# cgmb/euler

Hardware: AMD Instinct MI355X
Metric: cells*steps/sec of sim_step() (frames incl. the PCG pressure projection) + pressure-solve HBM GB/s vs roofline (higher is better)
Workload: dtype f64

## Files before the change

### euler_amd/csrc/driver.hip

```cpp
#include "euler_dev.h"
#include "k_mg.h"

#include <math.h>
#include <stdarg.h>
#include <stdlib.h>
#include <string.h>

#include <vector>

int eu_launch_build_system(euler_sim* S, float dt);
int eu_launch_velocity_update(euler_sim* S, float dt, int finish);
int eu_pressure_current(euler_sim* S);
int eu_unskew(euler_sim* S, const void* skew, void* rowmajor, int elem_bytes);
int eu_unskew_fluid(euler_sim* S, const double* skew, double* rowmajor);
double* eu_current_search_direction(euler_sim* S);
int eu_launch_tile_table(euler_sim* S);
int eu_skew(euler_sim* S, const void* rowmajor, void* skew, int elem_bytes);

static thread_local char g_err[512] = "";

void eu_set_error(const char* fmt, ...) {
  va_list ap;
  va_start(ap, fmt);
  vsnprintf(g_err, sizeof(g_err), fmt, ap);
// ... 105 lines not shown
  return EULER_OK;
}

bool eu_resident_eligible(const euler_sim* S) {
  if (S->res_disabled || S->cfg.resident == EULER_RESIDENT_OFF) return false;
  if (S->cfg.precond != EULER_PRECOND_IC0_TILE || S->tile_w != 16 || S->cfg.sweep_mode == EULER_SWEEP_SIMPLE || S->cfg.dot_mode != EULER_DOT_TREE) return false;
  if (S->has_comm || S->slab_on || S->p2p_on) return false;
  const int cap = eu_resident_capacity(const_cast<euler_sim*>(S), S->cfg.pcg_precision == EULER_PCG_F32);
  if (S->cfg.pcg_precision == EULER_PCG_F32) return cap > 0 && S->geom.nbands * (S->geom.T / 16) <= 4 * cap;
  return cap > 0;
}
extern "C" int euler_resident_info(euler_sim* S, uint64_t out[3]) {
  if (!S || !out) return EULER_EINVAL;
  out[0] = eu_resident_eligible(S) ? 1 : 0; out[1] = S->res_solves; out[2] = S->res_fallbacks;
  return EULER_OK;
}

extern "C" int euler_set_option(euler_sim* S, int32_t key, int64_t value) {
  if (!S || key <= 0 || key >= EULER_OPT__COUNT) { eu_set_error("euler_set_option: unknown key %d", (int)key); return EULER_EINVAL; }
  bool ok = true;
  const char* when = nullptr;
  switch (key) {
    case EULER_OPT_P_STEPS: ok = value == 2 || value == 4 || value == 8; break;
    case EULER_OPT_SA_RUN: ok = value == 8 || value == 16 || value == 32;
      if (ok && value != 8 && (S->has_comm || eu_is_two_level(S))) when = "on a handle without a communicator, in the parity or the plain tile-local mode (the others run runs of 8)";
      break;
    case EULER_OPT_RCCL_SMALL: ok = value >= 0 && value <= 2; if (S->rccl) when = "before euler_set_comm_rccl"; break;
    case EULER_OPT_RCCL_NO_EXCHANGE: ok = value == 0 || value == 1; if (S->rccl) when = "before euler_set_comm_rccl"; break;
    case EULER_OPT_SLAB_FUSION: ok = value == 0 || value == 1; if (S->p2p_on) when = "before euler_p2p_connect"; break;
    case EULER_OPT_RESIDENT_CAP: case EULER_OPT_GRID4_MIN_CELLS: case EULER_OPT_RESIDENT_FORCE_TIMEOUT: ok = value >= 0; break;
    case EULER_OPT_MG_SPLIT_LEVEL: ok = value >= -1 && value < 12; break;
    case EULER_OPT_PROFILE_STRIDE: ok = value >= 1 && value <= 1024; break;
    case EULER_OPT_MG_SPLIT_ACTIVE: ok = false; break;
    case EULER_OPT_ADVECT_RK2: ok = value == 0 || value == 1;
      if (ok && value == 1 && S->slab_on) when = "on a whole-grid handle (row slabs: the midpoint samples reach one row beyond the ghost rows)";
      break;
    case EULER_OPT_ADVECT_MACCORMACK: ok = value == 0 || value == 1;
      if (ok && value == 1 && S->slab_on) when = "on a whole-grid handle (row slabs: the correction reads the forward result one row beyond the own rows)";
      break;
    default: ok = value == 0 || value == 1; break;
  }
  if (!ok) { eu_set_error("euler_set_option: key %d does not take the value %lld", (int)key, (long long)value); return EULER_EINVAL; }
  if (when) { eu_set_error("euler_set_option: key %d must be set %s", (int)key, when); return EULER_ESTATE; }
  HIPCHK(hipStreamSynchronize(S->stream));
  if (key == EULER_OPT_ADVECT_MACCORMACK && value == 1 && !S->mc_u) {
    float *a = nullptr, *b = nullptr;
    const size_t bytes = S->C * sizeof(float);
    if (hipMalloc((void**)&a, bytes) != hipSuccess || hipMalloc((void**)&b, bytes) != hipSuccess || hipMemset(a, 0, bytes) != hipSuccess ||
        hipMemset(b, 0, bytes) != hipSuccess) {
      if (a) (void)hipFree(a);
      if (b) (void)hipFree(b);
      (void)hipGetLastError();
      eu_set_error("euler_set_option: EULER_OPT_ADVECT_MACCORMACK needs %zu bytes of scratch", 2 * bytes);
      return EULER_ENOMEM;
    }
    S->mc_u = a; S->mc_v = b;
    S->hbm_bytes += 2 * bytes;
  }
  if (key == EULER_OPT_P_STEPS || key == EULER_OPT_SA_RUN) {
    int rcp = eu_pressure_current(S);
    if (rcp) return rcp;
  }
  S->opt[key] = value;
  if (key == EULER_OPT_P_STEPS || key == EULER_OPT_SA_RUN) S->s_ring_n = 0;
  if (key == EULER_OPT_MG_SPLIT_LEVEL) { eu_mg_split_release(S); S->opt[EULER_OPT_MG_SPLIT_ACTIVE] = 0; }
  return EULER_OK;
// ... 925 lines not shown
```

### euler_amd/csrc/k_pcg.h

```cpp
#pragma once

#include "euler_dev.h"
#include "k_mg.h"

#define COMM_CALL(expr) do { if ((expr) != 0) { eu_set_error("communicator callback failed: %s", #expr); return EULER_ECOMM; } } while (0)
#define LOC(ptr) ((ptr) + S->e_lo)
enum { SW_FACTOR = 0, SW_FORWARD = 1, SW_BACKWARD = 2 };

int eu_launch_build_system(euler_sim* S, float dt);
int eu_launch_velocity_update(euler_sim* S, float dt, int finish);
int eu_launch_band_ranges(euler_sim* S);
int eu_launch_sweep(euler_sim* S, int op, int cls, int force, int fin_qq = -1);
int eu_launch_factor_tile(euler_sim* S, int force);
int eu_launch_precond_tile(euler_sim* S, int rupd, int sweeps, int fin_dot, int force, double alpha, bool r_only = false, int zform = -1);
int eu_launch_search_apply(euler_sim* S, int it);
int eu_launch_finish_p(euler_sim* S);
int eu_launch_dot(euler_sim* S, const double* a, const double* b, int fin_op, int force);
int eu_comm_exchange(euler_sim* S, double* send_lo, double* send_hi, double* recv_lo, double* recv_hi, int count, double* small, int nsmall);
int eu_comm_finish(euler_sim* S, int fin_op, int is_max, int force);
int eu_comm_halo_two(euler_sim* S, double* a, double* b);
bool tile_recompute(const euler_sim* S);
int p_steps(const euler_sim* S);

enum { FIN_SIGMA_INIT = 0, FIN_ALPHA, FIN_RNORM, FIN_BETA, FIN_STORE_ONLY, FIN_TO_COMM };
#define FIN_VIA_P2P 0x100

static inline bool tile_fused(const euler_sim* S) { return eu_is_tile(S) && S->cfg.sweep_mode != EULER_SWEEP_SIMPLE; }
static inline bool ghost_mode(const euler_sim* S) { return S->has_comm && !S->p2p_on && tile_fused(S); }
enum { XR_ZSEND_LO = 0, XR_ZSEND_HI, XR_ZRECV_LO, XR_ZRECV_HI, XR_GS_LO0, XR_GS_LO1, XR_GS_HI0, XR_GS_HI1 };
static inline double* xrow(const euler_sim* S, int k) { return S->xrows + (size_t)k * S->xrow_len; }
static inline int sa_run(const euler_sim* S) {
  if (S->opt[EULER_OPT_SA_RUN] != 8 && !S->has_comm && !eu_is_two_level(S)) return (int)S->opt[EULER_OPT_SA_RUN];
  return 8;
}
static inline bool tile_z_recompute(const euler_sim* S) {
  return tile_recompute(S) && tile_fused(S) && !eu_is_two_level(S) && S->tile_w == 16 && !S->has_comm && !S->slab_on && S->band_lo == 0 &&
         S->opt[EULER_OPT_TILE_STORE_Z] == 0 && S->chunk_list && S->tile_table;
}
static inline int fin_or_comm(const euler_sim* S, int fin_op) {
  return S->has_comm ? (S->p2p_on ? (fin_op | FIN_VIA_P2P) : (int)FIN_TO_COMM) : fin_op;
}

#ifdef __HIPCC__
#define RED_THREADS 1024
typedef double sw_d2 __attribute__((ext_vector_type(2)));

__device__ __forceinline__ bool pcg_idle(const PcgScalars* sc) { return sc->done || !sc->nonzero; }

#define DPP_WAVE_SHL1 0x130
#define DPP_WAVE_SHR1 0x138

template <int CTRL>
__device__ __forceinline__ double wave_shift_inject(double v, double edge) {
  const int lo = __builtin_amdgcn_update_dpp(__double2loint(edge), __double2loint(v), CTRL, 0xf, 0xf, false);
  const int hi = __builtin_amdgcn_update_dpp(__double2hiint(edge), __double2hiint(v), CTRL, 0xf, 0xf, false);
  return __hiloint2double(hi, lo);
}


__device__ __forceinline__ void pcg_scalar_step(PcgScalars* sc, int op, double v) {
  switch (op) {
    case FIN_SIGMA_INIT: sc->sigma = v; break;
    case FIN_ALPHA: sc->zs = v; sc->alpha_prev = sc->alpha; sc->alpha = sc->sigma / v; sc->alpha_hist[sc->iters & 7] = sc->alpha; sc->iters += 1; break;
    case FIN_RNORM: sc->rnorm = v; if (v <= sc->tol) sc->done = 1; break;
    case FIN_BETA: sc->sigma_new = v; sc->beta = v / sc->sigma; sc->sigma = v; break;
    case FIN_TO_COMM: sc->comm_val = v; if (sc->comm_slot) *sc->comm_slot = v; break;
    default: sc->sigma_new = v; break;
  }
}

template <int NT = RED_THREADS>
// ... 129 lines not shown
  unsigned int* qq_counter;
  PcgScalars* sc_w;
};

struct TileArgs {
  SkewGeom g;
  const uint8_t* mask;
  double* pre;
  double* r;
  const double* as;
  double* z;
  int band_lo, nb_local;
  int rupd;
  int sweeps;
  int fin_dot;
  int via;
  double* part_max; double* part_dot;
  unsigned int* counter;
  const unsigned int* list;
  const double* table;
  PcgScalars* sc;
  int force;
  double alpha_arg;
  double* pair_slot;
  double *zsend_lo, *zsend_hi;
  int edge_lo, edge_hi;
  int reverse;
  double* cpart;
  int cshift;
  int cmode, cnx, cny;
  const double *gs_lo, *gs_hi;
  int zform;
  double *zhalo, *zrows;
};

__device__ __forceinline__ double factor_step(double aa, double own, double nbv) {
  const double cl = -1.0 * own, cb = -1.0 * nbv;
  double e = aa - cl * cl - cb * cb;
  if (e < 0.25 * aa) e = (aa != 0.0) ? aa : 1.0;
  return 1.0 / sqrt(e);
}

template <int CTRL>
__device__ __forceinline__ double dpp_move(double v) {
  const int lo = __builtin_amdgcn_update_dpp(0, __double2loint(v), CTRL, 0xf, 0xf, true);
  const int hi = __builtin_amdgcn_update_dpp(0, __double2hiint(v), CTRL, 0xf, 0xf, true);
  return __hiloint2double(hi, lo);
}
__device__ __forceinline__ double group_sum(double v) {
  v = v + dpp_move<0xB1>(v);
  v = v + dpp_move<0x4E>(v);
  if (MG_LG == 8) v = v + dpp_move<0x141>(v);
  return v;
}
#endif
```

### euler_amd/csrc/k_pcg.hip

```cpp
#include "k_pcg.h"

#include <cmath>
#include <vector>

template <bool IS_MAX>
__global__ __launch_bounds__(RED_THREADS) void k_reduce_final(const double* __restrict__ partial, int n, PcgScalars* sc,
                                                              int op, int force) {
  if (!force && pcg_idle(sc)) return;
  double v = 0.0;
  for (int i = threadIdx.x; i < n; i += RED_THREADS) {
    const double w = partial[i];
    if (IS_MAX) v = w > v ? w : v; else v += w;
  }
  v = IS_MAX ? block_max(v) : block_sum(v);
  if (threadIdx.x == 0) pcg_scalar_step(sc, op, v);
}

template <bool EDGES>
__global__ __launch_bounds__(RED_THREADS) void k_dot_partial(const double* __restrict__ a, const double* __restrict__ b,
                                                             const uint8_t* __restrict__ mask, size_t S,
                                                             double* __restrict__ partial, PcgScalars* sc, int force,
                                                             unsigned int* counter, int fin_op, int TS, int nb_local, int edges) {
  if (!force && pcg_idle(sc)) return;
  const size_t chunk = (((S + gridDim.x - 1) / gridDim.x) + 1) & ~(size_t)1;
// ... 491 lines not shown
      S->prof_iter = -2;
      if (int rc = eu_launch_resident(S, cap_chunks)) return rc;
      HIPCHK(hipMemcpyAsync(S->sc_host, S->sc, sizeof(PcgScalars), hipMemcpyDeviceToHost, S->stream));
      HIPCHK(hipStreamSynchronize(S->stream));
      S->res_last_chunks = S->sc_host->n_chunks; S->res_have_last = 1;
      const int err = *S->res_err;
      if (err == 0) {
        if (S->sc_host->nonzero) { S->res_solves += 1; S->pcg_fields_resident = 1; }
        return eu_launch_velocity_update(S, dt, 0);
      }
      *S->res_err = 0;
      if (S->cfg.pcg_precision == EULER_PCG_F32 && err == 2) { eu_set_error("EULER_PCG_F32: the solve's active chunks do not fit the resident solver"); return EULER_EHIP; }
      if (err != 2) { S->res_fallbacks += 1; S->res_disabled = 1; }
      S->solve_seq -= 1;
      S->lean_ok = 0;
      S->res_skip_once = 1;
      *S->sc_host = v.prev;
      return eu_launch_project(S, dt);
    }
  }
  return EULER_OK;
}

static int project_first_direction(euler_sim* S, Solve& v) {
  int rc;
  const bool tile = tile_fused(S), two_level = tile && eu_is_two_level(S);
  if (two_level && S->has_comm && !(eu_is_mg(S) && ghost_mode(S) && S->slab_on)) {
    eu_set_error("coarse-correction preconditioners with several ranks: EULER_PRECOND_IC0_TILE_MG on row slabs without mailboxes only");
    return EULER_EINVAL;
  }
  if (two_level && (rc = eu_launch_coarse_setup(S))) return rc;
  if (two_level && (rc = eu_launch_coarse_consistent(S))) return rc;
  v.zr = tile && tile_z_begin(S);
  if (tile) {
    if ((rc = eu_launch_factor_tile(S, 0))) return rc;
    if ((rc = eu_launch_precond_tile(S, 0, 1, FIN_SIGMA_INIT, 0, 0.0))) return rc;
  } else {
  if (S->cfg.precond != EULER_PRECOND_JACOBI && (rc = eu_launch_sweep(S, SW_FACTOR, KC_PRECON_FACTOR, 0))) return rc;
  if ((rc = launch_precondition(S, 0, FIN_SIGMA_INIT))) return rc;
  }
  if ((rc = ring_begin(S))) return rc;
  if (first_direction_folded(S)) {
    const PcgScalars& ps = v.prev;
    if (ps.nonzero && !(std::isfinite(ps.alpha) && std::isfinite(ps.beta) && std::isfinite(ps.rnorm) && std::isfinite(ps.sigma) && std::isfinite(ps.zs)))
      for (int k = 0; k < S->s_ring_n; ++k) HIPCHK(hipMemsetAsync(S->s_ring[k] + S->skew_off, 0, S->Sw * sizeof(double), S->stream));
  }
  else if (two_level) { if ((rc = eu_launch_coarse_search_init(S))) return rc; }
  else
  LAUNCH(S, KC_UPDATE_SEARCH, k_update_search<true>, dim3(eu_blocks(S->e_cnt, 256 * 4, 4096)), dim3(256), LOC(S->s), LOC(S->z),
         LOC(S->cellmask), S->e_cnt, S->sc, 0, 0.0);
  if (S->has_comm && eu_p2p_has_neighbour_arrays(S)) {
    const int y0 = S->band_lo > 0 ? 64 * S->band_lo : -1, y1 = S->band_hi < S->geom.nbands ? 64 * S->band_hi - 1 : -1;
    LAUNCH(S, KC_UPDATE_SEARCH, k_publish_edge_rows, dim3((S->X + 255) / 256, 2), dim3(256), S->s, S->geom, y0, y1, S->sc);
  }
  if (S->s_ring_n == 2) HIPCHK(hipMemsetAsync(LOC(S->s2), 0, S->e_cnt * sizeof(double), S->stream));
  S->s_stale = 1;
  return EULER_OK;
}

static int project_iterate(euler_sim* S, Solve& v) {
  int rc;
  HIPCHK(hipMemcpyAsync(S->sc_host, S->sc, sizeof(PcgScalars), hipMemcpyDeviceToHost, S->stream));
  HIPCHK(hipStreamSynchronize(S->stream));
  const int poll = S->cfg.pcg_poll_interval > 0 ? S->cfg.pcg_poll_interval : 8;
  const int max_it = S->cfg.max_iterations;
  const bool tile = tile_fused(S), fold0 = first_direction_folded(S);
  int it = 0, chunk = 0;
  bool stop = !S->sc_host->nonzero;
  S->s_none = stop ? 1 : 0;
  while (it < max_it && !stop) {
    int chunk_end = it + poll;
    if (!v.drain_poll && v.pred_iters > 0 && it < v.pred_iters + poll && chunk_end > v.pred_iters - 2) {
      const int lo = v.pred_iters - 2 < chunk_end ? v.pred_iters - 2 : chunk_end;
      chunk_end = lo > it + 2 ? lo : it + 2;
    }
    if (chunk_end > max_it) chunk_end = max_it;
    for (; it < chunk_end; ++it) {
      S->prof_iter = it;
      const bool fused = it > 0 || fold0;
      if (it == 0 && fold0) { S->s = S->s_ring[S->s_ring_n - 1]; S->s2 = S->s_ring[0]; }
      if ((rc = fused ? eu_launch_search_apply(S, it) : launch_apply_a_and_alpha(S, 0))) return rc;
      if (tile) {
        S->prof_iter = it;
        const int nx = it + 1, steps = S->s_ring_n;
        const bool next_odd = !(nx >= steps && nx % steps == 0);
        const int zform = v.zr && it + 1 < max_it ? (it + 2 < max_it && next_odd ? 1 : 0) : -1;
        if ((rc = eu_launch_precond_tile(S, 1, it + 1 < max_it, FIN_BETA, 0, 0.0, false, zform))) return rc;
        S->z_halo_last = zform == 1;
        v.zr_ran = v.zr_ran || zform == 1;
        continue;
      }
      S->tile_as_override = fused ? S->q : S->z;
      rc = eu_launch_precond_tile(S, 1, 0, -1, 0, 0.0, true);
      S->tile_as_override = nullptr;
      if (rc) return rc;
      if (it + 1 < max_it) {
        S->prof_iter = it + 1;
        if ((rc = launch_precondition(S, 0, FIN_BETA))) return rc;
      }
    }
    if (it < max_it && v.drain_poll) {
      HIPCHK(hipMemcpyAsync(S->sc_host, S->sc, sizeof(PcgScalars), hipMemcpyDeviceToHost, S->stream));
      HIPCHK(hipStreamSynchronize(S->stream));
      stop = S->sc_host->done != 0;
    } else
    if (it < max_it) {
      const int slot = chunk & 1;
      if (chunk > 0) {
        HIPCHK(hipEventSynchronize(S->poll_event[slot ^ 1]));
        stop = S->poll_host[slot ^ 1].done != 0;
      }
      HIPCHK(hipMemcpyAsync(&S->poll_host[slot], S->sc, sizeof(PcgScalars), hipMemcpyDeviceToHost, S->stream));
      HIPCHK(hipEventRecord(S->poll_event[slot], S->stream));
      ++chunk;
    }
  }
  return EULER_OK;
}

// ... 85 lines not shown
```

### euler_amd/csrc/k_search.hip

```cpp
#include "k_pcg.h"

#include <type_traits>

#define SA_THREADS 256
struct SaPair { sw_d2 z, so; double ez0, es0, ez1, es1; };

__device__ __forceinline__ double pick3(int t, int tb1, int tb2, double v0, double v1, double v2) {
  double v = v0;
  v = t >= tb1 ? v1 : v;
  v = t >= tb2 ? v2 : v;
  return v;
}
template <int SLAB, int PMODE, int SA_RUN, int COARSE = 0, bool STORE = true, bool ZR = false>
__global__ __launch_bounds__(SA_THREADS, (COARSE == 2 && PMODE == 1 && SLAB == 0) ? 4 : 1) void k_search_apply(const double* __restrict__ s_old, const double* __restrict__ z,
                                                             double* __restrict__ s_new, double* __restrict__ out,
                                                             const uint8_t* __restrict__ mask, SkewGeom g,
                                                             double* __restrict__ partial, PcgScalars* sc, int force,
                                                             unsigned int* counter, int fin_op, SlabNeighbours nbr,
                                                             double* __restrict__ p, double* s_new_base, double* s_old_base,
                                                             const unsigned int* __restrict__ chunk_list,
                                                             CoarseRef cref, SaHist hist, ZrArgs zr) {
  static_assert(PMODE == 1 || PMODE == 2 || PMODE == 4 || PMODE == 8, "PMODE: p is left alone (1) or takes the N fmadds that are due (the ring's length)");
  static_assert(!ZR || (SLAB == 0 && SA_RUN == 8 && COARSE == 0), "ZR: one GPU, runs of one tile, no coarse part");
  __shared__ double s_cy[COARSE == 2 ? SA_THREADS / 64 : 1][COARSE == 2 ? MG_NI + 1 : 1][64];
  __shared__ double s_ce[COARSE == 2 ? SA_THREADS / 64 : 1][COARSE == 2 ? MG_NI + 1 : 1][64];
  if (!force && pcg_idle(sc)) return;
  __shared__ sw_d2 s_ztab[ZR ? 8 : 1][64];
  if (ZR) {
    for (int k = threadIdx.x; k < 8 * 64; k += SA_THREADS) (&s_ztab[0][0])[k] = reinterpret_cast<const sw_d2*>(zr.table)[k];
    __syncthreads();
  }
  const double beta = sc->beta;
  (void)s_new_base; (void)s_old_base;
  constexpr int NPA = PMODE >= 2 ? PMODE : 2;
  double al[NPA] = {};
  if (PMODE >= 2) {
    const int k = sc->iters;
#pragma unroll
    for (int j = 0; j < NPA; ++j) al[j] = sc->alpha_hist[(k - NPA + j) & 7];
  }
  const int lane = threadIdx.x & 63;
  const int TS = g.TS, npairs = TS / 2;
  const int nb_local = (int)(g.S / ((size_t)TS * 64));
  const int cpb = (npairs + SA_RUN - 1) / SA_RUN, total = nb_local * cpb;
  const int n_waves = gridDim.x * (SA_THREADS / 64);
  const bool edge_lane = lane == 0 || lane == 63;
  double t = 0.0;
  const bool listed = chunk_list != nullptr;
  const int ntb16 = g.T / 16;
  const int todo = listed ? (int)sc->n_chunks : total;
  typedef std::integral_constant<bool, true> yes_t;
  typedef std::integral_constant<bool, false> no_t;
  for (int i = blockIdx.x * (SA_THREADS / 64) + (threadIdx.x >> 6); i < todo; i += n_waves) {
    int c = i, per = cpb;
    bool interior = false;
    if (listed) { const unsigned int ent = chunk_list[i]; interior = (ent & EU_CHUNK_INTERIOR) != 0; c = (int)(ent & ~EU_CHUNK_INTERIOR); per = ntb16; }
    const int lb = c / per, P0 = (c % per) * SA_RUN, P1 = ZR ? P0 + SA_RUN : (P0 + SA_RUN < npairs ? P0 + SA_RUN : npairs);
    const size_t bbase = (size_t)lb * TS * 64 + 2 * lane;
    auto run = [&](auto full_tag) {
      constexpr bool FULL = decltype(full_tag)::value;
      unsigned int mm[SA_RUN];
      unsigned int any = 0;
#pragma unroll
      for (int j = 0; j < SA_RUN; ++j) {
        if (FULL) mm[j] = CM_INTERIOR | (CM_INTERIOR << 8);
        else mm[j] = P0 + j < P1 ? (unsigned int)*reinterpret_cast<const unsigned short*>(mask + bbase + (size_t)(P0 + j) * 128) : 0u;
        any |= mm[j];
      }
      if (!FULL && !listed && !__ballot(((any | (any >> 8)) & CM_FLUID) != 0)) return;
      sw_d2 zz[ZR ? SA_RUN : 1];
      if (ZR) {
        sw_d2 rr[SA_RUN], pp[SA_RUN];
#pragma unroll
        for (int j = 0; j < SA_RUN; ++j) {
          rr[j] = *reinterpret_cast<const sw_d2*>(zr.r + bbase + (size_t)(P0 + j) * 128);
          pp[j] = FULL ? s_ztab[j][lane] : *reinterpret_cast<const sw_d2*>(zr.pre + bbase + (size_t)(P0 + j) * 128);
        }
        double none = 0.0;
        tile_solve<2 * SA_RUN, false>(mm, rr, pp, zz, none);
      }
      const int ztile = P0 / SA_RUN;
      const bool up_remote = SLAB == 1 && nbr.z_up && lb + 1 == nb_local, dn_remote = SLAB == 1 && nbr.z_dn && lb == 0;
      const double* ez = lane == 0 ? (dn_remote ? nbr.z_dn : z) : (up_remote ? nbr.z_up : z);
      const double* es = lane == 0 ? (dn_remote ? nbr.s_dn : s_old) : (up_remote ? nbr.s_up : s_old);
      const bool remote = lane == 0 ? dn_remote : up_remote;
      const long long e0_base = lane == 0 ? ((long long)(lb - 1) * TS + 62) * 64 + 127 : ((long long)(lb + 1) * TS - 64) * 64 + 1;
      const long long e1_base = lane == 0 ? ((long long)(lb - 1) * TS + 64) * 64 + 126 : ((long long)(lb + 1) * TS - 62) * 64;
      const unsigned int vbit = lane == 0 ? CM_DOWN : CM_UP;
      const bool ghost = SLAB == 2 && (lane == 0 ? (nbr.zrow_dn != nullptr && lb == 0) : (nbr.zrow_up != nullptr && lb + 1 == nb_local));
      const double* gz = lane == 0 ? nbr.zrow_dn : nbr.zrow_up;
      const double* gs = lane == 0 ? nbr.srow_dn : nbr.srow_up;
      double* gsn = lane == 0 ? nbr.snew_dn : nbr.snew_up;
      const int gcol = lane == 0 ? 0 : -63;
      const double* zrow = ZR ? zr.rows + (long long)(lane == 0 ? 2 * lb - 1 : 2 * lb + 2) * zr.X : nullptr;
      double cy0 = 0.0, cy1 = 0.0, cy2 = 0.0, ce0 = 0.0, ce1 = 0.0, ce2 = 0.0;
      double (*cyv)[64] = s_cy[COARSE == 2 ? threadIdx.x >> 6 : 0];
      double (*cev)[64] = s_ce[COARSE == 2 ? threadIdx.x >> 6 : 0];
      int ctb1 = 0x7fffffff, ctb2 = 0x7fffffff, cJb = 0;
      (void)cJb;
      if (COARSE == 2) {
        cJb = (2 * (P0 - 1) - lane - MG_G0 / 2) >> MG_LOG;
        ctb1 = MG_G0 * (cJb + 1) + lane + MG_G0 / 2;
        const int row = (cref.band0 + lb) * 64 + lane;
        const int hi_ = cref.nx - 1;
        int i0, i1;
        double fy;
        mg_cell_w(row, cref.ny, i0, i1, fy);
        const double* y0 = cref.y + (size_t)i0 * cref.nx;
        const double* y1 = cref.y + (size_t)i1 * cref.nx;
#pragma unroll
        for (int q = 0; q <= MG_NI; ++q) { const int c = cJb + q < 0 ? 0 : (cJb + q < hi_ ? cJb + q : hi_); cyv[q][lane] = mg_rows(y0[c], y1[c], fy); }
#pragma unroll
        for (int q = 0; q <= MG_NI; ++q) cev[q][lane] = 0.0;
        if (edge_lane) {
          const int re = row + (lane == 0 ? -1 : 1);
          if (re >= 0 && re < MG_G0 * cref.ny) {
            mg_cell_w(re, cref.ny, i0, i1, fy);
            y0 = cref.y + (size_t)i0 * cref.nx; y1 = cref.y + (size_t)i1 * cref.nx;
#pragma unroll
            for (int q = 0; q <= MG_NI; ++q) { const int c = cJb + q < 0 ? 0 : (cJb + q < hi_ ? cJb + q : hi_); cev[q][lane] = mg_rows(y0[c], y1[c], fy); }
          }
        }
      }
      auto p0y = [&](int t, double (*av)[64]) __attribute__((always_inline)) {
        const double f = (double)((t - lane - MG_G0 / 2) & (MG_G0 - 1)) * (1.0 / MG_G0);
        int m = t >= ctb1 ? ((t - ctb1) >> MG_LOG) + 1 : 0;
        m = m < MG_NI - 1 ? m : MG_NI - 1;
        return mg_lerp_x(av[m][lane], av[m + 1][lane], f);
      };
      if (COARSE == 1) {
        const int xa = 2 * (P0 - 1) - lane, Ja = (xa > 0 ? xa : 0) >> cref.shift;
        const int row = (cref.band0 + lb) * 64 + lane;
        const size_t I = (size_t)(row >> cref.shift) * cref.nx;
        ctb1 = ((Ja + 1) << cref.shift) + lane;
        ctb2 = ((Ja + 2) << cref.shift) + lane;
        cy0 = Ja < cref.nx ? cref.y[I + Ja] : 0.0;
        cy1 = Ja + 1 < cref.nx ? cref.y[I + Ja + 1] : 0.0;
        cy2 = Ja + 2 < cref.nx ? cref.y[I + Ja + 2] : 0.0;
        if (edge_lane) {
          const int re = row + (lane == 0 ? -1 : 1);
          const bool inside = re >= 0 && (re >> cref.shift) < cref.ny;
          const size_t Ie = (size_t)((inside ? re : row) >> cref.shift) * cref.nx;
          ce0 = (inside && Ja < cref.nx) ? cref.y[Ie + Ja] : 0.0;
          ce1 = (inside && Ja + 1 < cref.nx) ? cref.y[Ie + Ja + 1] : 0.0;
          ce2 = (inside && Ja + 2 < cref.nx) ? cref.y[Ie + Ja + 2] : 0.0;
        }
      }
      auto load_pair = [&](int P, SaPair& d, unsigned int m) __attribute__((always_inline)) {
        d.ez0 = d.es0 = d.ez1 = d.es1 = 0.0;
        if (P < 0 || P >= npairs) { d.z = sw_d2{0.0, 0.0}; d.so = sw_d2{0.0, 0.0}; return; }
        if (ZR) {
          const int j = P - P0;
          if (j >= 0 && j < SA_RUN) d.z = zz[j >= 0 && j < SA_RUN ? j : 0];
          else if (j < 0) d.z = sw_d2{0.0, zr.halo[((size_t)lb * ntb16 + ztile - 1) * 128 + 64 + lane]};
          else d.z = sw_d2{ztile + 1 < ntb16 ? zr.halo[((size_t)lb * ntb16 + ztile + 1) * 128 + lane] : 0.0, 0.0};
        } else {
          d.z = *reinterpret_cast<const sw_d2*>(z + bbase + (size_t)P * 128);
        }
        d.so = *reinterpret_cast<const sw_d2*>(s_old + bbase + (size_t)P * 128);
        if (edge_lane) {
          if ((m & CM_FLUID) && (m & vbit)) {
            const long long k = e0_base + (long long)P * 128;
            if (ZR) { d.ez0 = zrow[2 * P + gcol]; d.es0 = s_old[k]; }
            else if (SLAB == 2 && ghost) { d.ez0 = gz[2 * P + gcol]; d.es0 = gs[2 * P + gcol]; }
            else if (SLAB == 1 && remote) { d.ez0 = ld_system(ez + k); d.es0 = ld_system(es + k); } else { d.ez0 = ez[k]; d.es0 = es[k]; }
          }
          if (((m >> 8) & CM_FLUID) && ((m >> 8) & vbit)) {
            const long long k = e1_base + (long long)P * 128;
            if (ZR) { d.ez1 = zrow[2 * P + 1 + gcol]; d.es1 = s_old[k]; }
            else if (SLAB == 2 && ghost) { d.ez1 = gz[2 * P + 1 + gcol]; d.es1 = gs[2 * P + 1 + gcol]; }
            else if (SLAB == 1 && remote) { d.ez1 = ld_system(ez + k); d.es1 = ld_system(es + k); } else { d.ez1 = ez[k]; d.es1 = es[k]; }
          }
          if (COARSE == 1) {
            d.ez0 = d.ez0 + pick3(2 * P, ctb1, ctb2, ce0, ce1, ce2);
            d.ez1 = d.ez1 + pick3(2 * P + 1, ctb1, ctb2, ce0, ce1, ce2);
          }
          if (COARSE == 2) {
            d.ez0 = d.ez0 + p0y(2 * P, cev);
            d.ez1 = d.ez1 + p0y(2 * P + 1, cev);
          }
        }
        if (COARSE == 1) {
          d.z.x = d.z.x + pick3(2 * P, ctb1, ctb2, cy0, cy1, cy2);
          d.z.y = d.z.y + pick3(2 * P + 1, ctb1, ctb2, cy0, cy1, cy2);
        }
        if (COARSE == 2) {
          d.z.x = d.z.x + p0y(2 * P, cyv);
          d.z.y = d.z.y + p0y(2 * P + 1, cyv);
        }
      };
      auto sprime = [&](const SaPair& d) __attribute__((always_inline)) { return sw_d2{d.z.x + beta * d.so.x, d.z.y + beta * d.so.y}; };
      SaPair A, B, Cn;
      load_pair(P0 - 1, A, 0u);
      load_pair(P0, B, mm[0]);
      load_pair(P0 + 1, Cn, SA_RUN > 1 ? mm[1] : 0u);
      double prev_y = sprime(A).y;
      sw_d2 cur = sprime(B);
#pragma unroll
      for (int j = 0; j < SA_RUN; ++j) {
        const int P = P0 + j;
        if (P < P1) {
          SaPair D;
          load_pair(P + 2 <= P1 ? P + 2 : -1, D, j + 2 < SA_RUN ? mm[j + 2] : 0u);
          const unsigned int m0 = mm[j] & 0xff, m1 = mm[j] >> 8;
          const sw_d2 nxt = sprime(Cn);
          const double e0 = B.ez0 + beta * B.es0, e1 = B.ez1 + beta * B.es1;
          if (SLAB == 2 && ghost && edge_lane) {
            if ((mm[j] & CM_FLUID) && (mm[j] & vbit)) gsn[2 * P + gcol] = e0;
            if (((mm[j] >> 8) & CM_FLUID) && ((mm[j] >> 8) & vbit)) gsn[2 * P + 1 + gcol] = e1;
          }
          const double dn0 = wave_shift_inject<DPP_WAVE_SHR1>(prev_y, e0), up0 = wave_shift_inject<DPP_WAVE_SHL1>(cur.y, e0);
          const double dn1 = wave_shift_inject<DPP_WAVE_SHR1>(cur.x, e1), up1 = wave_shift_inject<DPP_WAVE_SHL1>(nxt.x, e1);
          if ((m0 | m1) & CM_FLUID) {
            const size_t i = bbase + (size_t)P * 128;
            sw_d2 cc = B.so, o = {0.0, 0.0};
            if (PMODE >= 2) {
              sw_d2 pv = *reinterpret_cast<const sw_d2*>(p + i);
              constexpr int NP = PMODE >= 2 ? PMODE : 2;
              sw_d2 sv[NP];
              sv[0] = *reinterpret_cast<const sw_d2*>(s_new + i);
#pragma unroll
              for (int j = 1; j < NP - 1; ++j) sv[j] = *reinterpret_cast<const sw_d2*>(hist.s[j - 1] + i);
              sv[NP - 1] = B.so;
#pragma unroll
              for (int j = 0; j < NP; ++j) {
                if (m0 & CM_FLUID) pv.x = pv.x + sv[j].x * al[j];
                if (m1 & CM_FLUID) pv.y = pv.y + sv[j].y * al[j];
              }
              *reinterpret_cast<sw_d2*>(p + i) = pv;
            }
            if (m0 & CM_FLUID) cc.x = cur.x;
            if (m1 & CM_FLUID) cc.y = cur.y;
            if (m0 & CM_FLUID) {
              double v = (double)(int)(m0 >> CM_DIAG_SHIFT) * cc.x;
              v = v - ((m0 & CM_RIGHT) ? cc.y : 0.0);
              v = v - ((m0 & CM_UP) ? up0 : 0.0);
              v = v - ((m0 & CM_LEFT) ? prev_y : 0.0);
              v = v - ((m0 & CM_DOWN) ? dn0 : 0.0);
              o.x = v;
              t += v * cc.x;
            }
            if (m1 & CM_FLUID) {
              double v = (double)(int)(m1 >> CM_DIAG_SHIFT) * cc.y;
              v = v - ((m1 & CM_RIGHT) ? nxt.x : 0.0);
              v = v - ((m1 & CM_UP) ? up1 : 0.0);
              v = v - ((m1 & CM_LEFT) ? cc.x : 0.0);
              v = v - ((m1 & CM_DOWN) ? dn1 : 0.0);
              o.y = v;
              t += v * cc.y;
            }
            if ((m0 & m1) & CM_FLUID) *reinterpret_cast<sw_d2*>(s_new + i) = cc;
            else if (m0 & CM_FLUID) s_new[i] = cc.x;
            else s_new[i + 1] = cc.y;
            if (STORE) {
              if ((m0 & m1) & CM_FLUID) *reinterpret_cast<sw_d2*>(out + i) = o;
              else if (m0 & CM_FLUID) out[i] = o.x;
              else out[i + 1] = o.y;
            }
            if (SLAB == 1 && slab_edge_row(i, lane, TS, nb_local, (nbr.z_dn ? 1 : 0) | (nbr.z_up ? 2 : 0))) {
              if (m0 & CM_FLUID) st_system(s_new + i, cc.x);
              if (m1 & CM_FLUID) st_system(s_new + i + 1, cc.y);
            }
          }
// ... 32 lines not shown
    if (pmode == 8) return sa_pick_run<SLAB, COARSE, 8>(S, c, run, store);
    if (pmode == 4) return sa_pick_run<SLAB, COARSE, 4>(S, c, run, store);
  }
  if (pmode == 2) sa_pick_run<SLAB, COARSE, 2>(S, c, run, store); else sa_pick_run<SLAB, COARSE, 1>(S, c, run, store);
}
int eu_launch_search_apply(euler_sim* S, int it) {
  const bool seq = S->cfg.dot_mode == EULER_DOT_SEQUENTIAL && !S->has_comm;
  SlabNeighbours nbr = {nullptr, nullptr, nullptr, nullptr, S->band_hi - S->band_lo, nullptr, nullptr, nullptr, nullptr, nullptr, nullptr};
  const bool direct = S->has_comm && eu_p2p_has_neighbour_arrays(S);
  const bool ghost = ghost_mode(S);
  if (ghost) {
    const int c = S->gs_cur;
    if (S->band_lo > 0) { nbr.zrow_dn = xrow(S, XR_ZRECV_LO); nbr.srow_dn = xrow(S, XR_GS_LO0 + c); nbr.snew_dn = xrow(S, XR_GS_LO0 + (c ^ 1)); }
    if (S->band_hi < S->geom.nbands) { nbr.zrow_up = xrow(S, XR_ZRECV_HI); nbr.srow_up = xrow(S, XR_GS_HI0 + c); nbr.snew_up = xrow(S, XR_GS_HI0 + (c ^ 1)); }
    S->gs_cur = c ^ 1;
  } else if (direct) {
    eu_p2p_neighbour_arrays(S, &nbr.z_dn, &nbr.s_dn, &nbr.z_up, &nbr.s_up);
    if (nbr.z_dn) { nbr.z_dn += S->e_lo; nbr.s_dn += S->e_lo; }
    if (nbr.z_up) { nbr.z_up += S->e_lo; nbr.s_up += S->e_lo; }
  } else if (S->has_comm) {
    if (int rc = eu_comm_halo_two(S, S->z, S->s)) return rc;
  }
  const int steps = S->s_ring_n;
  const int pmode = (it >= steps && it % steps == 0) ? steps : 1;
  const bool mg = eu_is_mg(S);
  SaCall c = {S->geom, S->has_comm ? fin_or_comm(S, FIN_ALPHA) : (seq ? -1 : (int)FIN_ALPHA), nbr,
              {mg ? S->mg_x : S->cc_y, mg ? 0 : S->coarse_shift, mg ? S->mg_nx[0] : S->coarse_nx, mg ? S->mg_ny[0] : S->coarse_ny, S->band_lo},
              {{nullptr, nullptr, nullptr, nullptr, nullptr, nullptr}}, {S->r, S->precon, S->tile_table, S->zhalo, S->zrows, S->X}};
  c.gl.S = S->e_cnt;
  for (int j = 1; j + 1 < steps; ++j) c.hist.s[j - 1] = LOC(S->s_ring[j]);
  const int run = sa_run(S);
  const bool store = !tile_recompute(S);
  const bool coarse = eu_is_two_level(S) && tile_fused(S);
  if (S->z_halo_last) sa_launch<0, 1, 8, 0, false, true>(S, c);
  else if (coarse && ghost) sa_pick<2, 2>(S, c, pmode, run, store);
  else if (coarse && mg) sa_pick<0, 2>(S, c, pmode, run, store);
  else if (coarse) sa_pick<0, 1>(S, c, pmode, run, store);
  else if (ghost) sa_pick<2, 0>(S, c, pmode, run, store);
  else if (direct) sa_pick<1, 0>(S, c, pmode, run, store);
  else sa_pick<0, 0>(S, c, pmode, run, store);
  S->s = S->s_ring[it % steps]; S->s2 = S->s_ring[(it + 1) % steps];
  S->s_launched = it + 1;
  if (seq) eu_launch_dot(S, S->q, S->s, FIN_ALPHA, 0);
  return S->has_comm ? eu_comm_finish(S, FIN_ALPHA, 0, 0) : EULER_OK;
}
```

### euler_amd/csrc/k_tile.hip

```cpp
#include "k_pcg.h"

#include <type_traits>

#define PT_THREADS 256
__device__ __forceinline__ void tile_block_reduce(double& mx, double& sm) {
  __shared__ double s_mx[PT_THREADS / 64], s_sm[PT_THREADS / 64];
  mx = eu_wave_max(mx);
  sm = eu_wave_sum(sm);
  __syncthreads();
  if ((threadIdx.x & 63) == 0) { s_mx[threadIdx.x >> 6] = mx; s_sm[threadIdx.x >> 6] = sm; }
  __syncthreads();
  if (threadIdx.x == 0) {
    mx = s_mx[0]; sm = s_sm[0];
    for (int k = 1; k < PT_THREADS / 64; ++k) { mx = s_mx[k] > mx ? s_mx[k] : mx; sm += s_sm[k]; }
  }
}

__global__ __launch_bounds__(64) void k_tile_table(double* __restrict__ tab) {
  const int lane = threadIdx.x & 63;
  double own = 0.0, out = 0.0;
  sw_d2 pp[8];
#pragma unroll
  for (int j = 0; j < 16; ++j) {
    const double nbv = wave_shift_inject<DPP_WAVE_SHR1>(out, 0.0);
// ... 212 lines not shown
        double c0 = 0.0, c1 = 0.0, c2 = 0.0;
#pragma unroll
        for (int j = 0; j < W; ++j) {
          const int cm = (int)((mm[j >> 1] >> ((j & 1) * 8)) & 0xff);
          const double rv = (cm & CM_FLUID) ? ((j & 1) ? rr[j >> 1].y : rr[j >> 1].x) : 0.0;
          const int x = k * W + j - lane;
          const int b = ((x > 0 ? x : 0) >> a.cshift) - J0;
          c0 += b == 0 ? rv : 0.0; c1 += b == 1 ? rv : 0.0; c2 += b == 2 ? rv : 0.0;
        }
        c0 = eu_wave_sum(c0); c1 = eu_wave_sum(c1); c2 = eu_wave_sum(c2);
        if (lane == 0) { double* cp = a.cpart + (size_t)tile * 3; cp[0] = c0; cp[1] = c1; cp[2] = c2; }
      }
      if (RECOMP && a.rupd) {
        asm volatile("" ::: "memory");
#pragma unroll
        for (int P = 0; P < W / 2; ++P) pp[P] = FULL ? s_tab[P < TABP ? P : 0][lane] : *reinterpret_cast<const sw_d2*>(a.pre + base + P * 128);
      }
      tile_solve<W, true>(mm, rr, pp, qq, dsum);
      if (W == 16 && a.zform == 1) {
        double* h = a.zhalo + ((size_t)band * ntb + k) * 128;
        h[lane] = qq[0].x;
        h[64 + lane] = qq[W / 2 - 1].y;
        if (lane == 0 || lane == 63) {
          double* row = a.zrows + ((size_t)band * 2 + (lane == 63 ? 1 : 0)) * a.g.X;
#pragma unroll
          for (int j = 0; j < W; ++j) {
            const int x = k * W + j - lane;
            if (x >= 0 && x < a.g.X) row[x] = (j & 1) ? qq[j >> 1].y : qq[j >> 1].x;
          }
        }
      } else {
#pragma unroll
        for (int P = 0; P < W / 2; ++P) *reinterpret_cast<sw_d2*>(a.z + base + P * 128) = qq[P];
      }
      if (band == a.edge_lo || band == a.edge_hi) {
        const bool lo = band == a.edge_lo && lane == 0, hi = band == a.edge_hi && lane == 63;
#pragma unroll
        for (int j = 0; j < W; ++j) {
          const double zv = (j & 1) ? qq[j >> 1].y : qq[j >> 1].x;
          const int x_lo = k * W + j, x_hi = k * W + j - 63;
          if (lo && x_lo < a.g.X) a.zsend_lo[x_lo] = zv;
          if (hi && x_hi >= 0 && x_hi < a.g.X) a.zsend_hi[x_hi] = zv;
        }
      }
    };
    if (W == 16 && interior) run(yes_t()); else run(no_t());
  }
  tile_block_reduce(mx, dsum);
  __shared__ int am_last;
  if (threadIdx.x == 0) {
    __hip_atomic_store(reinterpret_cast<unsigned long long*>(&a.part_max[blockIdx.x]), (unsigned long long)__double_as_longlong(mx), __ATOMIC_RELAXED, __HIP_MEMORY_SCOPE_AGENT);
    __hip_atomic_store(reinterpret_cast<unsigned long long*>(&a.part_dot[blockIdx.x]), (unsigned long long)__double_as_longlong(dsum), __ATOMIC_RELAXED, __HIP_MEMORY_SCOPE_AGENT);
    asm volatile("s_waitcnt vmcnt(0)" ::: "memory");
    const unsigned int t = __hip_atomic_fetch_add(a.counter, 1u, __ATOMIC_RELAXED, __HIP_MEMORY_SCOPE_AGENT);
    am_last = t == gridDim.x - 1;
  }
  __syncthreads();
  if (!am_last) return;
  double vmax = 0.0, vsum = 0.0;
  for (unsigned int i = threadIdx.x; i < gridDim.x; i += PT_THREADS) {
    const double m = __longlong_as_double((long long)__hip_atomic_load(reinterpret_cast<unsigned long long*>(&a.part_max[i]), __ATOMIC_RELAXED, __HIP_MEMORY_SCOPE_AGENT));
    const double d = __longlong_as_double((long long)__hip_atomic_load(reinterpret_cast<unsigned long long*>(&a.part_dot[i]), __ATOMIC_RELAXED, __HIP_MEMORY_SCOPE_AGENT));
    vmax = m > vmax ? m : vmax; vsum += d;
  }
  tile_block_reduce(vmax, vsum);
  if (a.via == FIN_VIA_P2P) {
// ... 2 lines not shown
  }
  if (threadIdx.x == 0) {
    if (a.via == FIN_TO_COMM) { a.pair_slot[0] = vmax; a.pair_slot[1] = vsum; }
    else {
      if (a.rupd) pcg_scalar_step(a.sc, FIN_RNORM, vmax);
      if (a.fin_dot >= 0 && !(a.rupd && a.sc->done)) pcg_scalar_step(a.sc, a.fin_dot, vsum);
    }
    if (a.zform >= 0) a.sc->zfix = a.zform == 1 ? 1u : 0u;
    __hip_atomic_store(a.counter, 0u, __ATOMIC_RELAXED, __HIP_MEMORY_SCOPE_AGENT);
  }
}

__global__ void k_pair_fold(PcgScalars* sc, const double* __restrict__ pairs, int stride, int R, int rupd, int fin_dot, int force) {
  if (!force && pcg_idle(sc)) return;
  double vmax = 0.0, vsum = 0.0;
  for (int r = 0; r < R; ++r) { vmax = pairs[(size_t)stride * r] > vmax ? pairs[(size_t)stride * r] : vmax; vsum += pairs[(size_t)stride * r + 1]; }
  if (rupd) pcg_scalar_step(sc, FIN_RNORM, vmax);
  if (fin_dot >= 0 && !(rupd && sc->done)) pcg_scalar_step(sc, fin_dot, vsum);
}
static TileArgs make_tile_args(euler_sim* S, int force) {
  TileArgs a;
  a.g = S->geom; a.mask = S->cellmask; a.pre = S->precon; a.r = S->r; a.as = S->tile_as_override ? S->tile_as_override : S->q; a.z = S->z;
  a.band_lo = S->band_lo; a.nb_local = S->band_hi - S->band_lo;
  a.rupd = 0; a.sweeps = 1; a.fin_dot = -1;
  a.via = S->has_comm ? (S->p2p_on ? (int)FIN_VIA_P2P : (int)FIN_TO_COMM) : 0;
  a.part_max = S->partial; a.part_dot = S->partial2; a.counter = S->red_counter; a.sc = S->sc; a.force = force; a.alpha_arg = 0.0;
  a.pair_slot = S->pair_buf + 2 * (S->has_comm ? S->comm.rank : 0);
  a.list = !force ? S->chunk_list : nullptr;
  a.table = S->tile_table;
  a.zsend_lo = a.zsend_hi = nullptr; a.edge_lo = a.edge_hi = -1;
  a.reverse = S->opt[EULER_OPT_TILE_REVERSE] != 0;
  a.cpart = nullptr; a.cshift = 0; a.cmode = 0; a.cnx = a.cny = 0;
  a.gs_lo = a.gs_hi = nullptr;
  a.zform = -1; a.zhalo = S->zhalo; a.zrows = S->zrows;
  if (ghost_mode(S)) {
    if (S->band_lo > 0) { a.zsend_lo = xrow(S, XR_ZSEND_LO); a.edge_lo = S->band_lo; }
    if (S->band_hi < S->geom.nbands) { a.zsend_hi = xrow(S, XR_ZSEND_HI); a.edge_hi = S->band_hi - 1; }
  }
  return a;
}
static inline unsigned tile_blocks(const euler_sim* S, int w) {
  return eu_blocks((size_t)(S->band_hi - S->band_lo) * (S->geom.T / w), PT_THREADS / 64, 2048);
}
typedef void (*TileKernel)(TileArgs);
int eu_launch_factor_tile(euler_sim* S, int force) {
  const TileKernel k = S->tile_w == 8 ? k_factor_tile<8> : S->tile_w == 32 ? k_factor_tile<32> : k_factor_tile<16>;
  LAUNCH(S, KC_PRECON_FACTOR, k, dim3(tile_blocks(S, S->tile_w)), dim3(PT_THREADS), make_tile_args(S, force));
  return EULER_OK;
}
int eu_launch_precond_tile(euler_sim* S, int rupd, int sweeps, int fin_dot, int force, double alpha, bool r_only, int zform) {
  const bool seq = S->cfg.dot_mode == EULER_DOT_SEQUENTIAL && !S->has_comm;
  TileArgs a = make_tile_args(S, force);
  a.rupd = rupd; a.sweeps = sweeps; a.fin_dot = (seq || !sweeps) ? -1 : fin_dot; a.alpha_arg = alpha;
  a.zform = zform;
  const bool two_level = eu_is_two_level(S) && sweeps && !r_only && !force && a.list != nullptr;
  const int fin_real = a.fin_dot;
  if (two_level) {
    const bool mg = eu_is_mg(S);
    a.cpart = mg ? S->mg_part : S->cc_part; a.cshift = mg ? 0 : S->coarse_shift;
    a.cmode = mg ? 2 : 1; a.cnx = mg ? S->mg_nx[0] : 0; a.cny = mg ? S->mg_ny[0] : 0;
    if (a.fin_dot >= 0) a.fin_dot = FIN_STORE_ONLY;
  }
  double* xsmall = S->pair_buf;
  int nsmall = 2;
  bool split = false;
  if (two_level && a.via == FIN_TO_COMM) {
    split = eu_is_mg(S) && ghost_mode(S) && eu_mg_split(S);
    nsmall = eu_coarse_comm_slots(S);
    if (nsmall < 0) return EULER_ENOMEM;
    xsmall = S->mg_xbuf;
    a.pair_slot = xsmall + (size_t)S->comm.rank * nsmall;
    if (split) {
      if (a.zsend_lo) a.zsend_lo = eu_mg_split_msg(S, 0);
      if (a.zsend_hi) a.zsend_hi = eu_mg_split_msg(S, 1);
    }
  }
  const int w = r_only ? 16 : S->tile_w, cls = r_only ? KC_UPDATE_PR : zform == 2 ? KC_MISC : KC_PRECOND_TILE;
  const bool recomp = rupd && !force && tile_recompute(S) && (r_only ? S->tile_as_override == S->q : !S->tile_as_override);
  if (recomp) {
    a.as = S->s;
    if (ghost_mode(S)) {
      if (S->band_lo > 0) a.gs_lo = xrow(S, XR_GS_LO0 + S->gs_cur);
      if (S->band_hi < S->geom.nbands) a.gs_hi = xrow(S, XR_GS_HI0 + S->gs_cur);
    }
  }
  const TileKernel k = w == 8 ? k_precond_tile<8> : w == 32 ? k_precond_tile<32>
                     : a.cmode == 2 ? (recomp ? k_precond_tile<16, true, 2> : k_precond_tile<16, false, 2>)
// ... 24 lines not shown
```

Before: 195.8 million.

## Store initial search direction from precond tile and recompute z on flush steps

New measurement: 198.5 million, median of 6. No clear change (+1.4%).

```diff
diff --git a/euler_amd/csrc/driver.hip b/euler_amd/csrc/driver.hip
--- a/euler_amd/csrc/driver.hip
+++ b/euler_amd/csrc/driver.hip
@@ -161,6 +161,7 @@
     case EULER_OPT_MG_SPLIT_LEVEL: ok = value >= -1 && value < 12; break;
     case EULER_OPT_PROFILE_STRIDE: ok = value >= 1 && value <= 1024; break;
     case EULER_OPT_MG_SPLIT_ACTIVE: ok = false; break;
+    case EULER_OPT_TILE_STORE_Z: ok = value >= 0 && value <= 2; break;
     case EULER_OPT_ADVECT_RK2: ok = value == 0 || value == 1;
       if (ok && value == 1 && S->slab_on) when = "on a whole-grid handle (row slabs: the midpoint samples reach one row beyond the ghost rows)";
       break;
diff --git a/euler_amd/csrc/k_pcg.h b/euler_amd/csrc/k_pcg.h
--- a/euler_amd/csrc/k_pcg.h
+++ b/euler_amd/csrc/k_pcg.h
@@ -12,7 +12,7 @@
 int eu_launch_band_ranges(euler_sim* S);
 int eu_launch_sweep(euler_sim* S, int op, int cls, int force, int fin_qq = -1);
 int eu_launch_factor_tile(euler_sim* S, int force);
-int eu_launch_precond_tile(euler_sim* S, int rupd, int sweeps, int fin_dot, int force, double alpha, bool r_only = false, int zform = -1);
+int eu_launch_precond_tile(euler_sim* S, int rupd, int sweeps, int fin_dot, int force, double alpha, bool r_only = false, int zform = -1, double* s0 = nullptr);
 int eu_launch_search_apply(euler_sim* S, int it);
 int eu_launch_finish_p(euler_sim* S);
 int eu_launch_dot(euler_sim* S, const double* a, const double* b, int fin_op, int force);
@@ -35,8 +35,9 @@
 }
 static inline bool tile_z_recompute(const euler_sim* S) {
   return tile_recompute(S) && tile_fused(S) && !eu_is_two_level(S) && S->tile_w == 16 && !S->has_comm && !S->slab_on && S->band_lo == 0 &&
-         S->opt[EULER_OPT_TILE_STORE_Z] == 0 && S->chunk_list && S->tile_table;
-}
+         S->opt[EULER_OPT_TILE_STORE_Z] != 1 && S->chunk_list && S->tile_table;
+}
+static inline bool tile_z_flush_recompute(const euler_sim* S) { return S->opt[EULER_OPT_TILE_STORE_Z] == 0; }
 static inline int fin_or_comm(const euler_sim* S, int fin_op) {
   return S->has_comm ? (S->p2p_on ? (fin_op | FIN_VIA_P2P) : (int)FIN_TO_COMM) : fin_op;
 }
@@ -232,6 +233,7 @@
   const double *gs_lo, *gs_hi;
   int zform;
   double *zhalo, *zrows;
+  double* s0;
 };
 
 __device__ __forceinline__ double factor_step(double aa, double own, double nbv) {
diff --git a/euler_amd/csrc/k_pcg.hip b/euler_amd/csrc/k_pcg.hip
--- a/euler_amd/csrc/k_pcg.hip
+++ b/euler_amd/csrc/k_pcg.hip
@@ -547,21 +547,23 @@
   if (two_level && (rc = eu_launch_coarse_setup(S))) return rc;
   if (two_level && (rc = eu_launch_coarse_consistent(S))) return rc;
   v.zr = tile && tile_z_begin(S);
+  const bool s0_stored = tile && tile_z_recompute(S);
+  if (s0_stored && (rc = ring_begin(S))) return rc;
   if (tile) {
     if ((rc = eu_launch_factor_tile(S, 0))) return rc;
-    if ((rc = eu_launch_precond_tile(S, 0, 1, FIN_SIGMA_INIT, 0, 0.0))) return rc;
+    if ((rc = eu_launch_precond_tile(S, 0, 1, FIN_SIGMA_INIT, 0, 0.0, false, -1, s0_stored ? S->s : nullptr))) return rc;
   } else {
   if (S->cfg.precond != EULER_PRECOND_JACOBI && (rc = eu_launch_sweep(S, SW_FACTOR, KC_PRECON_FACTOR, 0))) return rc;
   if ((rc = launch_precondition(S, 0, FIN_SIGMA_INIT))) return rc;
   }
-  if ((rc = ring_begin(S))) return rc;
+  if (!s0_stored && (rc = ring_begin(S))) return rc;
   if (first_direction_folded(S)) {
     const PcgScalars& ps = v.prev;
     if (ps.nonzero && !(std::isfinite(ps.alpha) && std::isfinite(ps.beta) && std::isfinite(ps.rnorm) && std::isfinite(ps.sigma) && std::isfinite(ps.zs)))
       for (int k = 0; k < S->s_ring_n; ++k) HIPCHK(hipMemsetAsync(S->s_ring[k] + S->skew_off, 0, S->Sw * sizeof(double), S->stream));
   }
   else if (two_level) { if ((rc = eu_launch_coarse_search_init(S))) return rc; }
-  else
+  else if (!s0_stored)
   LAUNCH(S, KC_UPDATE_SEARCH, k_update_search<true>, dim3(eu_blocks(S->e_cnt, 256 * 4, 4096)), dim3(256), LOC(S->s), LOC(S->z),
          LOC(S->cellmask), S->e_cnt, S->sc, 0, 0.0);
   if (S->has_comm && eu_p2p_has_neighbour_arrays(S)) {
@@ -598,8 +600,8 @@
       if (tile) {
         S->prof_iter = it;
         const int nx = it + 1, steps = S->s_ring_n;
-        const bool next_odd = !(nx >= steps && nx % steps == 0);
-        const int zform = v.zr && it + 1 < max_it ? (it + 2 < max_it && next_odd ? 1 : 0) : -1;
+        const bool next_flush = nx >= steps && nx % steps == 0;
+        const int zform = v.zr && it + 1 < max_it ? (it + 2 < max_it && (!next_flush || tile_z_flush_recompute(S)) ? 1 : 0) : -1;
         if ((rc = eu_launch_precond_tile(S, 1, it + 1 < max_it, FIN_BETA, 0, 0.0, false, zform))) return rc;
         S->z_halo_last = zform == 1;
         v.zr_ran = v.zr_ran || zform == 1;
diff --git a/euler_amd/csrc/k_search.hip b/euler_amd/csrc/k_search.hip
--- a/euler_amd/csrc/k_search.hip
+++ b/euler_amd/csrc/k_search.hip
@@ -12,7 +12,7 @@
   return v;
 }
 template <int SLAB, int PMODE, int SA_RUN, int COARSE = 0, bool STORE = true, bool ZR = false>
-__global__ __launch_bounds__(SA_THREADS, (COARSE == 2 && PMODE == 1 && SLAB == 0) ? 4 : 1) void k_search_apply(const double* __restrict__ s_old, const double* __restrict__ z,
+__global__ __launch_bounds__(SA_THREADS, (COARSE == 2 && PMODE == 1 && SLAB == 0) ? 4 : (ZR && PMODE >= 2) ? 3 : 1) void k_search_apply(const double* __restrict__ s_old, const double* __restrict__ z,
                                                              double* __restrict__ s_new, double* __restrict__ out,
                                                              const uint8_t* __restrict__ mask, SkewGeom g,
                                                              double* __restrict__ partial, PcgScalars* sc, int force,
@@ -37,7 +37,10 @@
   if (PMODE >= 2) {
     const int k = sc->iters;
 #pragma unroll
-    for (int j = 0; j < NPA; ++j) al[j] = sc->alpha_hist[(k - NPA + j) & 7];
+    for (int j = 0; j < NPA; ++j) {
+      al[j] = sc->alpha_hist[(k - NPA + j) & 7];
+      if (ZR) al[j] = __hiloint2double(__builtin_amdgcn_readfirstlane(__double2hiint(al[j])), __builtin_amdgcn_readfirstlane(__double2loint(al[j])));
+    }
   }
   const int lane = threadIdx.x & 63;
   const int TS = g.TS, npairs = TS / 2;
@@ -68,6 +71,33 @@
         any |= mm[j];
       }
       if (!FULL && !listed && !__ballot(((any | (any >> 8)) & CM_FLUID) != 0)) return;
+      auto p_update = [&](size_t i, unsigned int m0, unsigned int m1, sw_d2 so) __attribute__((always_inline)) {
+        sw_d2 pv = *reinterpret_cast<const sw_d2*>(p + i);
+        constexpr int NP = PMODE >= 2 ? PMODE : 2;
+        sw_d2 sv[NP];
+        sv[0] = *reinterpret_cast<const sw_d2*>(s_new + i);
+#pragma unroll
+        for (int j = 1; j < NP - 1; ++j) sv[j] = *reinterpret_cast<const sw_d2*>(hist.s[j - 1] + i);
+        sv[NP - 1] = so;
+#pragma unroll
+        for (int j = 0; j < NP; ++j) {
+          if (m0 & CM_FLUID) pv.x = pv.x + sv[j].x * al[j];
+          if (m1 & CM_FLUID) pv.y = pv.y + sv[j].y * al[j];
+        }
+        *reinterpret_cast<sw_d2*>(p + i) = pv;
+      };
+      constexpr bool PFIRST = ZR && PMODE >= 2;
+      if (PFIRST) {
+        size_t pbase = bbase + (size_t)P0 * 128;
+        asm volatile("" : "+v"(pbase));
+#pragma unroll
+        for (int j = 0; j < SA_RUN; ++j) {
+          const unsigned int m0 = mm[j] & 0xff, m1 = mm[j] >> 8;
+          const size_t i = pbase + (size_t)j * 128;
+          if ((m0 | m1) & CM_FLUID) p_update(i, m0, m1, *reinterpret_cast<const sw_d2*>(s_old + i));
+        }
+        asm volatile("" ::: "memory");
+      }
       sw_d2 zz[ZR ? SA_RUN : 1];
       if (ZR) {
         sw_d2 rr[SA_RUN], pp[SA_RUN];
@@ -78,21 +108,25 @@
         }
         double none = 0.0;
         tile_solve<2 * SA_RUN, false>(mm, rr, pp, zz, none);
-      }
+        if (PFIRST) asm volatile("" ::: "memory");
+      }
+      int ln = lane;
+      if (PFIRST) asm volatile("" : "+v"(ln));
+      const bool edge_ln = ln == 0 || ln == 63;
       const int ztile = P0 / SA_RUN;
       const bool up_remote = SLAB == 1 && nbr.z_up && lb + 1 == nb_local, dn_remote = SLAB == 1 && nbr.z_dn && lb == 0;
-      const double* ez = lane == 0 ? (dn_remote ? nbr.z_dn : z) : (up_remote ? nbr.z_up : z);
-      const double* es = lane == 0 ? (dn_remote ? nbr.s_dn : s_old) : (up_remote ? nbr.s_up : s_old);
-      const bool remote = lane == 0 ? dn_remote : up_remote;
-      const long long e0_base = lane == 0 ? ((long long)(lb - 1) * TS + 62) * 64 + 127 : ((long long)(lb + 1) * TS - 64) * 64 + 1;
-      const long long e1_base = lane == 0 ? ((long long)(lb - 1) * TS + 64) * 64 + 126 : ((long long)(lb + 1) * TS - 62) * 64;
-      const unsigned int vbit = lane == 0 ? CM_DOWN : CM_UP;
-      const bool ghost = SLAB == 2 && (lane == 0 ? (nbr.zrow_dn != nullptr && lb == 0) : (nbr.zrow_up != nullptr && lb + 1 == nb_local));
-      const double* gz = lane == 0 ? nbr.zrow_dn : nbr.zrow_up;
-      const double* gs = lane == 0 ? nbr.srow_dn : nbr.srow_up;
-      double* gsn = lane == 0 ? nbr.snew_dn : nbr.snew_up;
-      const int gcol = lane == 0 ? 0 : -63;
-      const double* zrow = ZR ? zr.rows + (long long)(lane == 0 ? 2 * lb - 1 : 2 * lb + 2) * zr.X : nullptr;
+      const double* ez = ln == 0 ? (dn_remote ? nbr.z_dn : z) : (up_remote ? nbr.z_up : z);
+      const double* es = ln == 0 ? (dn_remote ? nbr.s_dn : s_old) : (up_remote ? nbr.s_up : s_old);
+      const bool remote = ln == 0 ? dn_remote : up_remote;
+      const long long e0_base = ln == 0 ? ((long long)(lb - 1) * TS + 62) * 64 + 127 : ((long long)(lb + 1) * TS - 64) * 64 + 1;
+      const long long e1_base = ln == 0 ? ((long long)(lb - 1) * TS + 64) * 64 + 126 : ((long long)(lb + 1) * TS - 62) * 64;
+      const unsigned int vbit = ln == 0 ? CM_DOWN : CM_UP;
+      const bool ghost = SLAB == 2 && (ln == 0 ? (nbr.zrow_dn != nullptr && lb == 0) : (nbr.zrow_up != nullptr && lb + 1 == nb_local));
+      const double* gz = ln == 0 ? nbr.zrow_dn : nbr.zrow_up;
+      const double* gs = ln == 0 ? nbr.srow_dn : nbr.srow_up;
+      double* gsn = ln == 0 ? nbr.snew_dn : nbr.snew_up;
+      const int gcol = ln == 0 ? 0 : -63;
+      const double* zrow = ZR ? zr.rows + (long long)(ln == 0 ? 2 * lb - 1 : 2 * lb + 2) * zr.X : nullptr;
       double cy0 = 0.0, cy1 = 0.0, cy2 = 0.0, ce0 = 0.0, ce1 = 0.0, ce2 = 0.0;
       double (*cyv)[64] = s_cy[COARSE == 2 ? threadIdx.x >> 6 : 0];
       double (*cev)[64] = s_ce[COARSE == 2 ? threadIdx.x >> 6 : 0];
@@ -152,13 +186,13 @@
         if (ZR) {
           const int j = P - P0;
           if (j >= 0 && j < SA_RUN) d.z = zz[j >= 0 && j < SA_RUN ? j : 0];
-          else if (j < 0) d.z = sw_d2{0.0, zr.halo[((size_t)lb * ntb16 + ztile - 1) * 128 + 64 + lane]};
-          else d.z = sw_d2{ztile + 1 < ntb16 ? zr.halo[((size_t)lb * ntb16 + ztile + 1) * 128 + lane] : 0.0, 0.0};
+          else if (j < 0) d.z = sw_d2{0.0, zr.halo[((size_t)lb * ntb16 + ztile - 1) * 128 + 64 + ln]};
+          else d.z = sw_d2{ztile + 1 < ntb16 ? zr.halo[((size_t)lb * ntb16 + ztile + 1) * 128 + ln] : 0.0, 0.0};
         } else {
           d.z = *reinterpret_cast<const sw_d2*>(z + bbase + (size_t)P * 128);
         }
         d.so = *reinterpret_cast<const sw_d2*>(s_old + bbase + (size_t)P * 128);
-        if (edge_lane) {
+        if (edge_ln) {
           if ((m & CM_FLUID) && (m & vbit)) {
             const long long k = e0_base + (long long)P * 128;
             if (ZR) { d.ez0 = zrow[2 * P + gcol]; d.es0 = s_old[k]; }
@@ -205,7 +239,7 @@
           const unsigned int m0 = mm[j] & 0xff, m1 = mm[j] >> 8;
           const sw_d2 nxt = sprime(Cn);
           const double e0 = B.ez0 + beta * B.es0, e1 = B.ez1 + beta * B.es1;
-          if (SLAB == 2 && ghost && edge_lane) {
+          if (SLAB == 2 && ghost && edge_ln) {
             if ((mm[j] & CM_FLUID) && (mm[j] & vbit)) gsn[2 * P + gcol] = e0;
             if (((mm[j] >> 8) & CM_FLUID) && ((mm[j] >> 8) & vbit)) gsn[2 * P + 1 + gcol] = e1;
           }
@@ -214,21 +248,7 @@
           if ((m0 | m1) & CM_FLUID) {
             const size_t i = bbase + (size_t)P * 128;
             sw_d2 cc = B.so, o = {0.0, 0.0};
-            if (PMODE >= 2) {
-              sw_d2 pv = *reinterpret_cast<const sw_d2*>(p + i);
-              constexpr int NP = PMODE >= 2 ? PMODE : 2;
-              sw_d2 sv[NP];
-              sv[0] = *reinterpret_cast<const sw_d2*>(s_new + i);
-#pragma unroll
-              for (int j = 1; j < NP - 1; ++j) sv[j] = *reinterpret_cast<const sw_d2*>(hist.s[j - 1] + i);
-              sv[NP - 1] = B.so;
-#pragma unroll
-              for (int j = 0; j < NP; ++j) {
-                if (m0 & CM_FLUID) pv.x = pv.x + sv[j].x * al[j];
-                if (m1 & CM_FLUID) pv.y = pv.y + sv[j].y * al[j];
-              }
-              *reinterpret_cast<sw_d2*>(p + i) = pv;
-            }
+            if (PMODE >= 2 && !PFIRST) p_update(i, m0, m1, B.so);
             if (m0 & CM_FLUID) cc.x = cur.x;
             if (m1 & CM_FLUID) cc.y = cur.y;
             if (m0 & CM_FLUID) {
@@ -327,7 +347,12 @@
   const int run = sa_run(S);
   const bool store = !tile_recompute(S);
   const bool coarse = eu_is_two_level(S) && tile_fused(S);
-  if (S->z_halo_last) sa_launch<0, 1, 8, 0, false, true>(S, c);
+  if (S->z_halo_last) {
+    if (pmode == 8) sa_launch<0, 8, 8, 0, false, true>(S, c);
+    else if (pmode == 4) sa_launch<0, 4, 8, 0, false, true>(S, c);
+    else if (pmode == 2) sa_launch<0, 2, 8, 0, false, true>(S, c);
+    else sa_launch<0, 1, 8, 0, false, true>(S, c);
+  }
   else if (coarse && ghost) sa_pick<2, 2>(S, c, pmode, run, store);
   else if (coarse && mg) sa_pick<0, 2>(S, c, pmode, run, store);
   else if (coarse) sa_pick<0, 1>(S, c, pmode, run, store);
diff --git a/euler_amd/csrc/k_tile.hip b/euler_amd/csrc/k_tile.hip
--- a/euler_amd/csrc/k_tile.hip
+++ b/euler_amd/csrc/k_tile.hip
@@ -268,6 +268,10 @@
       } else {
 #pragma unroll
         for (int P = 0; P < W / 2; ++P) *reinterpret_cast<sw_d2*>(a.z + base + P * 128) = qq[P];
+        if (W == 16 && a.s0) {
+#pragma unroll
+          for (int P = 0; P < W / 2; ++P) *reinterpret_cast<sw_d2*>(a.s0 + base + P * 128) = qq[P];
+        }
       }
       if (band == a.edge_lo || band == a.edge_hi) {
         const bool lo = band == a.edge_lo && lane == 0, hi = band == a.edge_hi && lane == 63;
@@ -336,7 +340,7 @@
   a.reverse = S->opt[EULER_OPT_TILE_REVERSE] != 0;
   a.cpart = nullptr; a.cshift = 0; a.cmode = 0; a.cnx = a.cny = 0;
   a.gs_lo = a.gs_hi = nullptr;
-  a.zform = -1; a.zhalo = S->zhalo; a.zrows = S->zrows;
+  a.zform = -1; a.zhalo = S->zhalo; a.zrows = S->zrows; a.s0 = nullptr;
   if (ghost_mode(S)) {
     if (S->band_lo > 0) { a.zsend_lo = xrow(S, XR_ZSEND_LO); a.edge_lo = S->band_lo; }
     if (S->band_hi < S->geom.nbands) { a.zsend_hi = xrow(S, XR_ZSEND_HI); a.edge_hi = S->band_hi - 1; }
@@ -352,11 +356,11 @@
   LAUNCH(S, KC_PRECON_FACTOR, k, dim3(tile_blocks(S, S->tile_w)), dim3(PT_THREADS), make_tile_args(S, force));
   return EULER_OK;
 }
-int eu_launch_precond_tile(euler_sim* S, int rupd, int sweeps, int fin_dot, int force, double alpha, bool r_only, int zform) {
+int eu_launch_precond_tile(euler_sim* S, int rupd, int sweeps, int fin_dot, int force, double alpha, bool r_only, int zform, double* s0) {
   const bool seq = S->cfg.dot_mode == EULER_DOT_SEQUENTIAL && !S->has_comm;
   TileArgs a = make_tile_args(S, force);
   a.rupd = rupd; a.sweeps = sweeps; a.fin_dot = (seq || !sweeps) ? -1 : fin_dot; a.alpha_arg = alpha;
-  a.zform = zform;
+  a.zform = zform; a.s0 = s0;
   const bool two_level = eu_is_two_level(S) && sweeps && !r_only && !force && a.list != nullptr;
   const int fin_real = a.fin_dot;
   if (two_level) {
```
